# zsc/ARTalk

Measured on AMD Instinct MI355X. Metric: motion frames/sec (25 fps clips) at batch=32 per GPU, higher is better.
Workload: dtype f32 (operands split into 2 fp16, 3 fp16 MFMA products per fp32 product, fp32 accumulate)

## Files before the change

artalk_amd/capi.py:

```python
from __future__ import annotations

import ctypes as C
import os

from .config import ARTalkConfig

_HERE = os.path.dirname(os.path.abspath(__file__))
LIB_PATH = os.environ.get("ARTALK_LIB") or os.path.join(_HERE, "libartalk_hip.so")

OK, EINVAL, EKEY, EMISSING, EHIP, ESTATE, ECAPACITY, EBUSY = 0, -1, -2, -3, -4, -5, -6, -7
DTYPE_F32, DTYPE_I64 = 0, 1

SYMBOLS = [
    "artalk_create", "artalk_destroy", "artalk_last_error", "artalk_set_tensor", "artalk_finalize_weights",
    "artalk_reserve", "artalk_workspace_bytes", "artalk_weight_bytes", "artalk_infer", "artalk_get_status", "artalk_poll_status", "artalk_last_ticket", "artalk_get_status_of", "artalk_style_encode", "artalk_stream_begin", "artalk_stream_chunk", "artalk_stream_end", "artalk_savgol", "artalk_flame_create", "artalk_flame_verts", "artalk_flame_destroy", "artalk_flame_last_error",
    "artalk_set_profiling", "artalk_get_profile", "artalk_get_kernel_sums", "artalk_set_graphs", "artalk_graph_count", "artalk_set_cu_mask", "artalk_set_audit", "artalk_get_audit", "artalk_calibrate", "artalk_reset_scales", "artalk_get_scales", "artalk_scale_sites", "artalk_get_site_scales", "artalk_set_site_scales", "artalk_set_tap", "artalk_tap_layout", "artalk_set_precision",
    "artalk_op_gemm", "artalk_op_gemm_ex", "artalk_op_gemm_bf16", "artalk_op_gemm_f16s", "artalk_op_pack_split", "artalk_op_gemm_f16s_packed", "artalk_op_release_scratch", "artalk_op_gemm_p8_plan", "artalk_op_create_masked_stream", "artalk_op_destroy_stream", "artalk_op_mfma_f32_peak", "artalk_op_layernorm", "artalk_op_attention", "artalk_op_w2v_front", "artalk_op_resample_mean", "artalk_op_pool_silu",
    "artalk_op_bsq_history",
    "artalk_sessions_reserve", "artalk_session_open", "artalk_session_step", "artalk_session_close", "artalk_session_count",
    "artalk_op_pack_split_ex", "artalk_op_layernorm_ex", "artalk_op_gemm_f16s_packed_ex", "artalk_op_gemm_f16s_ex", "artalk_op_attention_ex", "artalk_op_w2v_front_ex", "artalk_op_pool_silu_ex", "artalk_op_posconv_p8_ex",
    "artalk_op_bsq_history_ex", "artalk_op_ar_bits_next", "artalk_op_vq_embed", "artalk_op_ar_begin", "artalk_op_dec_input", "artalk_op_dec_finish", "artalk_op_enc_input_zero", "artalk_op_style_input", "artalk_op_add_row", "artalk_op_style_finish", "artalk_op_broadcast16", "artalk_op_session_gather", "artalk_op_session_scatter", "artalk_op_absmax",
]


class ArtalkConfigStruct(C.Structure):
    _fields_ = [
        ("ar_depth", C.c_int32), ("ar_heads", C.c_int32),
        ("vae_depth", C.c_int32), ("vae_heads", C.c_int32), ("vae_hidden", C.c_int32),
        ("code_dim", C.c_int32), ("motion_dim", C.c_int32),
        ("n_levels", C.c_int32), ("patch_nums", C.c_int32 * 8),
        ("w2v_layers", C.c_int32), ("w2v_hidden", C.c_int32), ("w2v_heads", C.c_int32), ("w2v_ffn", C.c_int32),
        ("w2v_n_conv", C.c_int32), ("w2v_conv_kernel", C.c_int32 * 8), ("w2v_conv_stride", C.c_int32 * 8),
        ("w2v_conv_dim", C.c_int32),
        ("w2v_pos_kernel", C.c_int32), ("w2v_pos_groups", C.c_int32),
        ("w2v_ln_eps", C.c_float),
        ("style_dim", C.c_int32), ("style_heads", C.c_int32), ("style_layers", C.c_int32), ("style_ffn", C.c_int32),
        ("style_len", C.c_int32),
    ]


def config_struct(cfg: ARTalkConfig) -> ArtalkConfigStruct:
    w = cfg.w2v
    if w.get("feat_extract_norm", "layer") != "layer" or not w.get("do_stable_layer_norm", True) or not w.get("conv_bias", True):
        raise ValueError("only the XLS-R style wav2vec2 (layer-norm conv stack, stable layer norm, conv bias) is supported")
# ... 177 lines not shown
        L.artalk_op_w2v_front_ex.restype = i32
        L.artalk_op_pool_silu_ex.argtypes = [vp, i32, i32, i32, vp, i32, i32, vp, vp]
        L.artalk_op_pool_silu_ex.restype = i32
        L.artalk_op_posconv_p8_ex.argtypes = [vp, vp, vp, vp, vp, i32, i32, i32, i32, i32, vp, vp]
        L.artalk_op_posconv_p8_ex.restype = i32
    if hasattr(L, "artalk_op_ar_bits_next"):
        for name, args in (
                ("bsq_history_ex", [vp, vp, vp, vp, i32, vp, vp]),
                ("ar_bits_next", [vp, vp, vp, vp, i32, i32, vp, vp]),
                ("vq_embed", [vp, i32, vp, vp, vp, vp, i32, i32, vp, vp, i32, vp]),
                ("ar_begin", [vp, vp, vp, vp, i32, vp]),
                ("dec_input", [vp, vp, vp, vp, vp, i32, vp]),
                ("dec_finish", [vp, vp, vp, vp, vp, i64, i32, vp, i32, vp, vp]),
                ("enc_input_zero", [vp, vp, vp, vp, i32, vp]),
                ("style_input", [vp, vp, vp, vp, i32, vp]),
                ("add_row", [vp, vp, i32, i32, vp]),
                ("style_finish", [vp, vp, vp, vp, vp, vp, i32, vp, i64, vp]),
                ("broadcast16", [vp, vp, i64, i32, vp]),
                ("session_gather", [vp, vp, vp, vp, i32, i32, i32, i32, vp]),
                ("session_scatter", [vp, vp, vp, vp, i32, i32, i32, i32, i32, vp]),
                ("absmax", [vp, i32, i32, i64, i32, i32, i32, i32, vp, vp])):
            f = getattr(L, "artalk_op_" + name)
            f.argtypes, f.restype = args, i32
    _lib = L
    return L


def ptr(t):
    return None if t is None else C.c_void_p(t.data_ptr())


def current_stream_ptr():
    import torch
    return C.c_void_p(torch.cuda.current_stream().cuda_stream)
```

artalk_amd/csrc/ar_glue.hip:

```cpp
#include "common.h"
#include <cmath>
#include <mutex>
#include <set>

namespace artalk {

constexpr int T100 = 100;
constexpr int CD = 32;
constexpr int NLV = 5;
__constant__ int c_pn[NLV];
__constant__ int c_off[NLV + 1];
__constant__ int c_up_i0[4][T100];
__constant__ int c_up_i1[4][T100];
__constant__ float c_up_w1[4][T100];
__constant__ float c_hq;

static const int h_pn[NLV] = {1, 5, 25, 50, 100};

int init_ms_tables() {
    static std::mutex mu;
    static std::set<int> ready;
    int dev = -1;
    if (hipGetDevice(&dev) != hipSuccess) return -1;
    std::lock_guard<std::mutex> lock(mu);
// ... 95 lines not shown
        if (status && !(isfinite(l[0]) && isfinite(l[1]))) atomicOr(status, 1);
        bits[((long)b * 181 + off + i) * CD + c] = (uint8_t)bit;
        hs[idx] = bit ? c_hq : -c_hq;
    }
    if (p >= NLV - 1) return;
    __syncthreads();
    float* fg = fhat + (long)b * T100 * CD;
    for (int idx = tid; idx < T100 * CD; idx += BITS_NT) {
        const int t = idx / CD, c = idx % CD;
        const float v = fg[idx] + up_lin(hs, p, t, c);
        fg[idx] = v;
        fs[idx] = v;
    }
    __syncthreads();
    const int pn2 = c_pn[p + 1];
    for (int idx = tid; idx < pn2 * CD; idx += BITS_NT)
        nextfeat[(long)b * pn2 * CD + idx] = area_pool(fs, pn2, idx / CD, idx % CD);
}
void launch_ar_bits_next(const float* logits, uint8_t* bits, float* fhat, float* nextfeat, int B, int level, hipStream_t s, int* status) {
    ARTALK_LAUNCH(ar_bits_kernel, dim3(B), dim3(BITS_NT), 0, s, logits, bits, fhat, nextfeat, level, status);
}

constexpr int VQ_TOK = 16;
__global__ __launch_bounds__(256) void vq_embed_kernel(const float* __restrict__ feat, int n, const float* __restrict__ We,
                                                       const float* __restrict__ be, const float* __restrict__ pos,
                                                       float* __restrict__ X, int xrows, int xoff,
                                                       const float* __restrict__ style_cond, const float* __restrict__ pos0, int E) {
    __shared__ float f[VQ_TOK][CD];
    const int i0 = blockIdx.x * VQ_TOK, b = blockIdx.y, tid = threadIdx.x;
    if (blockIdx.x == 0 && style_cond) {
        for (int e = tid; e < E; e += 256) X[((long)b * xrows) * E + e] = style_cond[(long)b * E + e] + pos0[e];
    }
    const int nt = min(VQ_TOK, n - i0);
    for (int idx = tid; idx < VQ_TOK * CD; idx += 256) f[idx / CD][idx % CD] = idx < nt * CD ? feat[((long)b * n + i0) * CD + idx] : 0.f;
    constexpr int EPT = 3;
    float w[EPT][CD], bias[EPT], pv[EPT][VQ_TOK];
#pragma unroll
    for (int k = 0; k < EPT; ++k) {
        const int e = tid + k * 256;
        const bool ok = e < E;
#pragma unroll
        for (int c4 = 0; c4 < CD / 4; ++c4) {
            f32x4 t = {0.f, 0.f, 0.f, 0.f};
            if (ok) t = *reinterpret_cast<const f32x4*>(We + (long)e * CD + 4 * c4);
            w[k][4 * c4] = t[0]; w[k][4 * c4 + 1] = t[1]; w[k][4 * c4 + 2] = t[2]; w[k][4 * c4 + 3] = t[3];
        }
        bias[k] = ok ? be[e] : 0.f;
#pragma unroll
        for (int t = 0; t < VQ_TOK; ++t) pv[k][t] = (ok && t < nt) ? pos[(long)(i0 + t) * E + e] : 0.f;
    }
    __syncthreads();
#pragma unroll
    for (int k = 0; k < EPT; ++k) {
        const int e = tid + k * 256;
        if (e >= E) break;
#pragma unroll
        for (int t0 = 0; t0 < VQ_TOK; t0 += 4) {
            float acc[4] = {0.f, 0.f, 0.f, 0.f};
#pragma unroll
            for (int c = 0; c < CD; ++c)
#pragma unroll
                for (int u = 0; u < 4; ++u) acc[u] = fmaf(w[k][c], f[t0 + u][c], acc[u]);
#pragma unroll
            for (int u = 0; u < 4; ++u)
                if (t0 + u < nt) X[((long)b * xrows + xoff + i0 + t0 + u) * E + e] = (acc[u] + bias[k]) + pv[k][t0 + u];
        }
    }
}
void launch_vq_embed(const float* feat, int n, const float* We, const float* be, const float* pos, float* X, int xrows,
                     int xoff, const float* style_cond, const float* pos0, int B, hipStream_t s) {
    ARTALK_LAUNCH(vq_embed_kernel, dim3((n + VQ_TOK - 1) / VQ_TOK, B), dim3(256), 0, s, feat, n, We, be, pos, X, xrows, xoff,
                       style_cond, pos0, 768);
}

__global__ __launch_bounds__(256) void dec_input_kernel(const float* __restrict__ prev_fdec, const float* __restrict__ fhat,
                                                        const uint8_t* __restrict__ bits, const float* __restrict__ dpos,
                                                        float* __restrict__ X) {
    const int b = blockIdx.x;
    for (int idx = blockIdx.y * 256 + threadIdx.x; idx < 2 * T100 * CD; idx += gridDim.y * 256) {
        const int t = idx / CD, c = idx % CD;
        float v;
        if (t < T100) {
            v = prev_fdec[(long)b * T100 * CD + idx];
        } else {
            const int tt = t - T100;
            const float h = bits[((long)b * 181 + 81 + tt) * CD + c] ? c_hq : -c_hq;
            v = fhat[(long)b * T100 * CD + tt * CD + c] + h;
        }
        X[(long)b * 2 * T100 * CD + idx] = v + dpos[idx];
    }
}
void launch_dec_input(const float* prev_fdec, const float* fhat, const uint8_t* bits, const float* dpos, float* X, int B,
                      hipStream_t s) {
    ARTALK_LAUNCH(dec_input_kernel, dim3(B, 8), dim3(256), 0, s, prev_fdec, fhat, bits, dpos, X);
}
// ... 257 lines not shown
```

artalk_amd/csrc/engine.hip:

```cpp
#include "kernels.h"
#include "../../include/artalk_hip.h"

#include <hip/hip_ext.h>
#include <rocprofiler-sdk-roctx/roctx.h>

#include <algorithm>
#include <cmath>
#include <cstdio>
#include <cstdlib>
#include <cstring>
#include <map>
#include <set>
#include <string>
#include <vector>

using namespace artalk;

namespace artalk {
thread_local KernelTimer* g_ktimer = nullptr;
bool ktimer_events(hipEvent_t* e0, hipEvent_t* e1) {
    KernelTimer* t = g_ktimer;
    if (!t) return false;
    while (t->pool.size() < t->used + 2) {
        hipEvent_t e = nullptr;
// ... 88 lines not shown
    int64_t weight_bytes = 0;
    struct PackRange { const float* base; int64_t n; unsigned int* packed; uint16_t* bf16; };
    std::vector<PackRange> wranges;
    int precision = 0;
    bool have_bf16 = false;
    int splitk_tiles = 192, splitk_target = 384;
    bool audit = false;
    unsigned int* audit_vals = nullptr;
    std::vector<std::string> audit_names;
    std::map<std::string, int> audit_index;
    std::vector<int*> audit_exp;
    SiteExps ex;
    int scales_changed = 0;
    struct Site { std::string name; int* ex; };
    std::vector<Site> sites;
    std::map<const int*, int> site_of;
    bool stream_scales_ended = false;
    struct InitHistory { uint8_t* bits = nullptr; float *fdec = nullptr, *msfeat = nullptr; bool valid = false; } init_hist[3];
    void invalidate_init_hist() { for (auto& ih : init_hist) ih.valid = false; }
    float* tap = nullptr; int tap_B = 0, tap_maxch = 0, tap_chunk = 0;
    std::vector<uint32_t> cu_mask;
    int n_cus = 0;
    int stream_B = 0;
    static constexpr int kSessBlock = 32;
    struct Sessions {
        std::vector<float*> blocks;
        std::vector<int64_t> owner;
        std::map<int64_t, int> open;
        std::set<int64_t> ended_by_scales;
        int64_t next_id = 1;
    } sess;
    int64_t sess_slot_floats() const { return kE + (int64_t)kNTok * kE + 100LL * cfg.code_dim; }
    float* sess_slot(int i) const { return sess.blocks[i / kSessBlock] + (int64_t)(i % kSessBlock) * sess_slot_floats(); }
    Workspace* view = nullptr;
    bool sticky_error = false;
    int n_conv = 0; int conv_T[8]{}; int conv_S[8]{};
    int Tw = 0, Ts = 0;
    int ada_n = 0;
    int pn[kMaxLv]{}, off[kMaxLv + 1]{};
    float *conv0_w = nullptr, *conv_b[8]{}, *conv_lnw[8]{}, *conv_lnb[8]{}, *conv_w[8]{};
    float *fp_lnw = nullptr, *fp_lnb = nullptr, *fp_w = nullptr, *fp_b = nullptr;
    float *pos_w = nullptr, *pos_b = nullptr, *enc_lnw = nullptr, *enc_lnb = nullptr;
    std::vector<W2VLayer> w2v;
    float *ada_w = nullptr, *ada_b = nullptr;
    float *ar_qkv_w = nullptr, *ar_qkv_b = nullptr;
    std::vector<ARLayer> ar;
// ... 508 lines not shown
        SiteExps::VAE& E = m->ex.vae[sd][i];
        layernorm(w.vh, w.vln, L.lnw, L.lnb, M, H, 1e-5f, ACT_NONE, s, p8, w.status, 0, 0, E.ln);
        audit(m, w.vln, M, H, H, p8, s, &E.ln);
        linear(m, w.vln, H, L.qkv_w, nullptr, w.vqkv, 3 * H, M, 3 * H, H, ACT_NONE, nullptr, s, AP | (p8 ? LF_C_P8 : 0), nullptr, E.ln, E.qkv);
        AttnArgs a;
        a.qkv_p8 = p8; a.qkv_exp = E.qkv; a.o_exp = E.attn;
        a.Q = w.vqkv; a.K = w.vqkv + H; a.V = w.vqkv + 2 * H; a.ldq = a.ldk = a.ldv = 3 * H;
        a.q_bstride = a.k_bstride = a.v_bstride = (long)T * 3 * H;
        a.O = w.vatt; a.ldo = H; a.o_bstride = (long)T * H;
        a.B = B; a.H = c.vae_heads; a.HD = H / c.vae_heads; a.Lq = T; a.Lk = T;
        a.scale = 1.0f / std::sqrt((float)H);
        audit(m, w.vqkv, M, 3 * H, 3 * H, p8, s, &E.qkv);
        a.split_q = split; a.split_k = split; a.out_p8 = p8; a.split16 = p8; a.status = p8 ? w.status : nullptr; a.cus = m->n_cus;
        launch_attention(a, s);
        audit(m, w.vatt, M, H, H, p8, s, &E.attn);
        linear(m, w.vatt, H, L.out_w, L.out_b, w.vh, H, M, H, H, ACT_NONE, w.vh, s, AP, p8 ? w.vln : nullptr, E.attn, E.resid);
        audit(m, p8 ? w.vln : w.vh, M, H, H, p8, s, &E.resid);
        linear(m, p8 ? w.vln : w.vh, H, L.m1_w, L.m1_b, w.vmlp, F, M, F, H, ACT_GELU_TANH, nullptr, s, p8 ? (LF_A_P8 | LF_C_P8) : 0, nullptr, E.resid, E.mlp);
        audit(m, w.vmlp, M, F, F, p8, s, &E.mlp);
        linear(m, w.vmlp, F, L.m2_w, L.m2_b, w.vh, H, M, H, F, ACT_NONE, w.vh, s, AP, nullptr, E.mlp);
    }
}

void run_reencode(artalk_model* m, int B, hipStream_t s) {
    const artalk_config& c = m->cfg;
    Workspace& w = m->view ? *m->view : m->ws;
    const int H = c.vae_hidden, T = 100;
    Range r_re("artalk.vae.reencode_bsq");
    kbucket(m, KB_REENC);
    audit(m, w.enc_in, B * T, 128, 128, false, s, &m->ex.vae_enc_in);
    linear(m, w.enc_in, 128, m->enc.in_w, m->enc.in_b, w.vh, H, B * T, H, 128, ACT_LEAKY02, nullptr, s, 0, nullptr, m->ex.vae_enc_in);
    run_vae_stack(m, m->enc, B, T, 0, s);
    linear(m, w.vh, H, m->enc.out_w, m->enc.out_b, w.enc_out, c.code_dim, B * T, c.code_dim, H, ACT_NONE, nullptr, s, LF_EXACT);
    launch_bsq_history(w.enc_out, w.hist_bits, w.prev_fdec, w.msfeat, B, s, w.status);
    launch_vq_embed(w.msfeat, kNTok - 1, m->vq_w, m->vq_b, m->prev_lvl_pos + kE, w.prev_in, kNTok, 1, w.style_cond,
                    m->prev_lvl_pos, B, s);
}

int run_init_history(artalk_model* m, int B, hipStream_t s) {
    const artalk_config& c = m->cfg;
    struct Restore { artalk_model* m; ~Restore() { kbucket(m, KB_OTHER); } } restore{m};
    Workspace& w = m->ws;
    artalk_model::InitHistory& ih = m->init_hist[m->precision];
    const long nb = (long)kNTok * c.code_dim, nf = 100L * c.code_dim * 4, nm = 180L * c.code_dim * 4;
    if (!ih.valid) {
        if (!ih.bits) {
            ih.bits = dalloc<uint8_t>(m, nb); ih.fdec = dalloc<float>(m, nf / 4); ih.msfeat = dalloc<float>(m, nm / 4);
            if (!ih.bits || !ih.fdec || !ih.msfeat) return fail(m, ARTALK_EHIP, "hipMalloc failed for the initial-history cache");
            HIPCHK(m, hipDeviceSynchronize());
        }
        launch_enc_input_zero(m->vae_mean, m->vae_std, m->enc_pos, w.enc_in, 1, s);
        run_reencode(m, 1, s);
        HIPCHK(m, hipMemcpyAsync(ih.bits, w.hist_bits, nb, hipMemcpyDeviceToDevice, s));
        HIPCHK(m, hipMemcpyAsync(ih.fdec, w.prev_fdec, nf, hipMemcpyDeviceToDevice, s));
        HIPCHK(m, hipMemcpyAsync(ih.msfeat, w.msfeat, nm, hipMemcpyDeviceToDevice, s));
        int flags[4] = {0, 0, 0, 0};
        HIPCHK(m, hipMemcpyAsync(flags, w.status, sizeof(int), hipMemcpyDeviceToHost, s));
        HIPCHK(m, hipStreamSynchronize(s));
        ih.valid = flags[0] == 0;
    }
    launch_broadcast16(ih.bits, w.hist_bits, nb, B, s);
    launch_broadcast16(ih.fdec, w.prev_fdec, nf, B, s);
    launch_broadcast16(ih.msfeat, w.msfeat, nm, B, s);
    launch_vq_embed(w.msfeat, kNTok - 1, m->vq_w, m->vq_b, m->prev_lvl_pos + kE, w.prev_in, kNTok, 1, w.style_cond, m->prev_lvl_pos, B, s);
    return ARTALK_OK;
}

void run_chunk_body(artalk_model* m, int B, hipStream_t s, int n_reencode = -1) {
    struct BodyScope { artalk_model* m; BodyScope(artalk_model* x) : m(x) { m->in_body = true; } ~BodyScope() { m->in_body = false; } } scope(m);
    const artalk_config& c = m->cfg;
    Workspace& w = m->view ? *m->view : m->ws;
    const long ldada = m->ada_n;
    const long cache_l = (long)w.maxB * 2 * kNTok * 3 * kE;
    const int p8 = m->precision == 1 ? 1 : 0;
    kbucket(m, KB_AR_MISC);
    tap_copy(m, TAP_PREV_IN, 0, w.prev_in, kNTok, kE, B, s);
    roctxRangePushA("artalk.ar.history_kv");
    SiteExps& ex = m->ex;
    if (p8) launch_pack_split(w.prev_in, reinterpret_cast<unsigned int*>(w.prev_in_p8), (long)B * kNTok * kE, false, s, w.status, ex.hist_tok);
    audit(m, p8 ? w.prev_in_p8 : w.prev_in, B * kNTok, kE, kE, p8, s, &ex.hist_tok);
    {
        GemmArgs g;
        g.A = p8 ? w.prev_in_p8 : w.prev_in; g.a_packed = p8; g.a_exp = ex.hist_tok;
        g.lda = kE; g.W = m->ar_qkv_w + (long)kE * kE; g.ldw = kE; g.bias = m->ar_qkv_b + kE;
        g.C = w.cache + kE; g.ldc = 3 * kE; g.cmap = rowmap(kNTok, 2 * kNTok, 0);
        g.M = B * kNTok; g.N = c.ar_depth * 2 * kE; g.K = kE;
        g.ngrp = 2 * kE; g.grpW = (long)3 * kE * kE; g.grpB = 3 * kE; g.grpC = cache_l;
        g.Wp = packed_of(m, g.W);
        if (p8 && gemm_p8_eligible(g)) {
            gemm(m, g, s);
        } else {
            for (int l = 0; l < c.ar_depth; ++l) {
                const ARLayer& L = m->ar[l];
                GemmArgs q = g;
                q.Wp = nullptr; q.ngrp = 0; q.grpW = q.grpB = q.grpC = 0;
                q.W = L.qkv_w + (long)kE * kE; q.bias = L.qkv_b + kE; q.C = w.cache + l * cache_l + kE; q.N = 2 * kE;
                gemm(m, q, s);
            }
        }
    }
    roctxRangePop();
    launch_ar_begin(w.style_cond, m->lvl_pos, w.x, w.fhat, B, s);
// ... 38 lines not shown
            a.B = B; a.H = c.ar_heads; a.HD = kE / c.ar_heads; a.Lq = pn; a.Lk = kNTok + off + pn; a.scale = 1.0f;
            a.l2norm = 1; a.qscale = L.qscale; a.out_p8 = p8; a.split16 = p8; a.status = p8 ? w.status : nullptr; a.o_exp = E.attn;
            launch_attention(a, s);
            audit(m, w.attn_out, M, kE, kE, p8, s, &E.attn);
            GemmArgs pj;
            pj.A = w.attn_out; pj.lda = kE; pj.W = L.proj_w; pj.ldw = kE; pj.bias = L.proj_b; pj.C = w.x; pj.ldc = kE;
            pj.gate = ada; pj.ldg = ldada; pj.gmap = amap; pj.R = w.x; pj.ldr = kE; pj.M = M; pj.N = kE; pj.K = kE; pj.a_packed = p8; pj.a_exp = E.attn;
            const LnArgs n2 = ln_args(l, 1);
            if (!gemm(m, pj, s, &n2)) launch_layernorm(n2, s);
            audit(m, w.xmod, M, kE, kE, p8, s, &E.ln2);
            linear(m, w.xmod, kE, L.ffn1_w, L.ffn1_b, w.ffn_h, 4 * kE, M, 4 * kE, kE, ACT_GELU_TANH, nullptr, s, p8 ? (LF_A_P8 | LF_C_P8) : 0, nullptr, E.ln2, E.ffn);
            audit(m, w.ffn_h, M, 4 * kE, 4 * kE, p8, s, &E.ffn);
            GemmArgs f2;
            f2.A = w.ffn_h; f2.lda = 4 * kE; f2.W = L.ffn2_w; f2.ldw = 4 * kE; f2.bias = L.ffn2_b; f2.C = w.x; f2.ldc = kE;
            f2.gate = ada + kE; f2.ldg = ldada; f2.gmap = amap; f2.R = w.x; f2.ldr = kE; f2.M = M; f2.N = kE; f2.K = 4 * kE; f2.a_packed = p8; f2.a_exp = E.ffn;
            const LnArgs nn = ln_args(l + 1, 0);
            have_ln = gemm(m, f2, s, &nn);
            if (l == 0) tap_copy(m, TAP_BLK0_OUT, off, w.x, pn, kE, B, s);
            if (l == c.ar_depth - 1) tap_copy(m, TAP_BLKL_OUT, off, w.x, pn, kE, B, s);
        }
        if (!have_ln) launch_layernorm(ln_args(c.ar_depth, 0), s);
        linear(m, w.xmod, kE, m->logits_w, m->logits_b, w.logits, 2 * c.code_dim, M, 2 * c.code_dim, kE, ACT_NONE, nullptr, s, LF_EXACT);
        tap_copy(m, TAP_LOGITS, off, w.logits, pn, 2 * c.code_dim, B, s);
        launch_ar_bits_next(w.logits, w.bits, w.fhat, w.nextfeat, B, p, s, w.status);
        if (p + 1 < c.n_levels)
            launch_vq_embed(w.nextfeat, m->pn[p + 1], m->vq_w, m->vq_b, m->lvl_pos + (long)m->off[p + 1] * kE, w.x, m->pn[p + 1], 0,
                            nullptr, nullptr, B, s);
    }
    stage_mark(m, s, PB_AR);
    const int H = c.vae_hidden;
    roctxRangePushA("artalk.vae.decode");
    kbucket(m, KB_VAE_DEC);
    launch_dec_input(w.prev_fdec, w.fhat, w.bits, m->dec_pos, w.dec_x, B, s);
    audit(m, w.dec_x, B * 200, c.code_dim, c.code_dim, false, s, &ex.vae_dec_in);
    linear(m, w.dec_x, c.code_dim, m->dec.in_w, m->dec.in_b, w.vh, H, B * 200, H, c.code_dim, ACT_LEAKY02, nullptr, s, 0, nullptr, ex.vae_dec_in);
    run_vae_stack(m, m->dec, B, 200, 100, s);
    audit(m, w.vh, B * 200, H, H, false, s, &ex.vae_dec_head);
    linear(m, w.vh, H, m->dec.out_w, m->dec.out_b, w.dec_out, c.motion_dim, B * 200, c.motion_dim, H, ACT_NONE, nullptr, s, 0, nullptr, ex.vae_dec_head);
    tap_copy(m, TAP_DEC_OUT, 0, w.dec_out, 200, c.motion_dim, B, s);
    launch_dec_finish(w.dec_out, m->vae_mean, m->vae_std, m->enc_pos, w.motion_chunk, 100L * c.motion_dim, 0, w.enc_in, B, s, w.status);
    roctxRangePop();
    if (n_reencode < 0 || n_reencode > B) n_reencode = B;
    if (n_reencode > 0) run_reencode(m, n_reencode, s);
    stage_mark(m, s, PB_VAE);
}

Workspace clip_view(const artalk_model* m, int b0, int branch) {
    const artalk_config& c = m->cfg;
    Workspace v = m->ws;
    const long b = b0;
// ... 137 lines not shown
    return ARTALK_OK;
}
int publish_status(artalk_model* m, hipStream_t s) {
    const int slot = (int)(m->ticket % artalk_model::kStatusSlots);
    if (m->ticket >= artalk_model::kStatusSlots) HIPCHK(m, hipEventSynchronize(m->status_ev[slot]));
    HIPCHK(m, hipMemcpyAsync(m->h_status + slot, m->ws.status, sizeof(int), hipMemcpyDeviceToHost, s));
    HIPCHK(m, hipEventRecord(m->status_ev[slot], s));
    ++m->ticket;
    m->status_pending = true;
    HIPCHK(m, hipGetLastError());
    return ARTALK_OK;
}

int reserve(artalk_model* m, int maxB, int maxC) {
    const artalk_config& c = m->cfg;
    if (maxB <= m->ws.maxB && maxC <= m->ws.maxC) return ensure_stage(m, m->ws.maxB, m->ws.maxC);
    maxB = std::max(maxB, m->ws.maxB); maxC = std::max(maxC, m->ws.maxC);
    (void)hipDeviceSynchronize();
    drop_graphs(m);
    for (void* p : m->ws_allocs) if (p) (void)hipFree(p);
    m->ws_allocs.clear();
    m->ws = Workspace();
    m->stream_B = 0; m->stream_scales_ended = false;
    m->status_pending = false;
    Workspace& w = m->ws;
    const int CD = c.w2v_conv_dim, Hs = c.w2v_hidden;
    w.maxB = maxB; w.maxC = maxC; w.G = std::min(maxC, 96);
    auto F = [&](int64_t n) { w.bytes += n * 4; return dalloc_in<float>(m->ws_allocs, n); };
    const int G = w.G;
    w.src_off = dalloc_in<long>(m->ws_allocs, maxC);
    w.xnorm = F((int64_t)G * kSamplesPerChunk);
    w.convA = F(((int64_t)G * m->conv_S[0] + 16) * CD);
    w.convB = F(((int64_t)G * m->conv_S[1] + 16) * CD);
    const int64_t M = (int64_t)G * m->Ts;
    w.h0 = F(M * Hs); w.h1 = F(M * Hs); w.xln = F(M * Hs); w.qkv = F(M * 3 * Hs); w.att = F(M * Hs); w.ffn = F(M * c.w2v_ffn);
    w.silu_cond = F((int64_t)maxC * kNTok * kCond);
    w.ada = F((int64_t)maxB * kNTok * m->ada_n);
    w.style_cond = F((int64_t)maxB * kE);
    w.prev_in = F((int64_t)maxB * kNTok * kE); w.prev_in_p8 = F((int64_t)maxB * kNTok * kE);
    w.cache = F((int64_t)c.ar_depth * maxB * 2 * kNTok * 3 * kE);
    w.x = F((int64_t)maxB * 100 * kE); w.xmod = F((int64_t)maxB * 100 * kE); w.attn_out = F((int64_t)maxB * 100 * kE);
    w.ffn_h = F((int64_t)maxB * 100 * 4 * kE); w.logits = F((int64_t)maxB * 100 * 2 * c.code_dim);
    w.splitk_floats = (int64_t)8 << 20; w.splitk = F(w.splitk_floats); w.splitk_b[0] = w.splitk;
    for (int i = 1; i < 4; ++i) w.splitk_b[i] = F(w.splitk_floats);
    w.fhat = F((int64_t)maxB * 100 * c.code_dim); w.nextfeat = F((int64_t)maxB * 100 * c.code_dim);
    w.bits = dalloc_in<uint8_t>(m->ws_allocs, (int64_t)maxB * kNTok * c.code_dim);
// ... 96 lines not shown
    Workspace& w = m->ws;
    if (!has_style) style_motion_dev = nullptr;
    if (style_motion_dev) {
        std::memcpy(stg->has, has_style, (size_t)B);
        HIPCHK(m, hipMemcpyAsync(w.has_style, stg->has, B, hipMemcpyHostToDevice, s));
    }
    HIPCHK(m, hipEventRecord(stg->done, s));
    stg->used = true;
    HIPCHK(m, hipMemsetAsync(w.status, 0, 4 * sizeof(int), s));
    stage_mark(m, s, PB_OTHER);
    run_style(m, style_motion_dev, B, s, encode_style);
    stage_mark(m, s, PB_STYLE);
    return ARTALK_OK;
}
int chunk_step(artalk_model* m, hipStream_t s, int cond_row0, int Bn, int n_next, int tap_chunk, float* out_motion_dev, int64_t out_stride) {
    Workspace& w = m->ws;
    m->tap_chunk = tap_chunk;
    roctxRangePushA("artalk.ar.adaln_table");
    kbucket(m, KB_ADA);
    linear(m, w.silu_cond + (long)cond_row0 * kNTok * kCond, kCond, m->ada_w, m->ada_b, w.ada, m->ada_n, Bn * kNTok, m->ada_n, kCond,
           ACT_NONE, nullptr, s, m->precision == 1 ? LF_A_P8 : 0, nullptr, m->ex.silu_cond);
    roctxRangePop();
    stage_mark(m, s, PB_ADA);
    if (body_uses_graphs(m)) {
        Range r_body("artalk.body.graph");
        if (int rc = run_body(m, Bn, s, n_next)) return rc;
        stage_mark(m, s, PB_AR);
    } else {
        if (int rc = run_body(m, Bn, s, n_next)) return rc;
    }
    const size_t mrow = (size_t)100 * m->cfg.motion_dim * 4;
    HIPCHK(m, hipMemcpy2DAsync(out_motion_dev, (size_t)out_stride * 4, w.motion_chunk, mrow, mrow, Bn, hipMemcpyDeviceToDevice, s));
    return ARTALK_OK;
}

SessionRows session_rows(const artalk_model* m) {
    const Workspace& w = m->ws;
    SessionRows r;
    r.style = reinterpret_cast<uint4*>(w.style_cond); r.prev_in = reinterpret_cast<uint4*>(w.prev_in); r.prev_fdec = reinterpret_cast<uint4*>(w.prev_fdec);
    r.s16 = kE / 4; r.p16 = kNTok * kE / 4; r.f16 = 100 * m->cfg.code_dim / 4;
    return r;
}
int grow_sessions(artalk_model* m, int64_t n_slots) {
    artalk_model::Sessions& ss = m->sess;
    if (m->cfg.code_dim % 4) return fail(m, ARTALK_EINVAL, "sessions need a code_dim that is a multiple of 4 (16-byte rows)");
    while ((int64_t)ss.owner.size() < n_slots) {
        void* p = nullptr;
        HIPCHK(m, hipMalloc(&p, (size_t)artalk_model::kSessBlock * m->sess_slot_floats() * sizeof(float)));
        ss.blocks.push_back(static_cast<float*>(p));
        ss.owner.resize(ss.owner.size() + artalk_model::kSessBlock, 0);
    }
    return ARTALK_OK;
}
// ... 546 lines not shown
            if (ss.ended_by_scales.count(ids[i]))
                return fail(m, ARTALK_ESTATE, "session " + std::to_string(ids[i]) + ": the site scales changed since artalk_session_open; open the session again");
            return fail(m, ARTALK_EINVAL, "artalk_session_step: " + std::to_string(ids[i]) + " is not an open session");
        }
        if (!seen.insert(ids[i]).second) return fail(m, ARTALK_EINVAL, "artalk_session_step: session " + std::to_string(ids[i]) + " is listed twice");
        slot[i] = it->second;
    }
    hipStream_t s;
    if (int rc = call_stream(m, stream, &s)) return rc;
    if (n > m->ws.maxB || n > m->ws.maxC) { if (int rc = reserve(m, n, n)) return rc; }
    Workspace& w = m->ws;
    artalk_model::Stage* stg = nullptr;
    if (int rc = next_stage(m, &stg)) return rc;
    for (int b = 0; b < n; ++b) stg->src[b] = (long)b * chunk_stride;
    HIPCHK(m, hipMemcpyAsync(w.src_off, stg->src, n * sizeof(long), hipMemcpyHostToDevice, s));
    if (int rc = stage_session_slots(m, s, stg, slot.data(), n)) return rc;
    HIPCHK(m, hipEventRecord(stg->done, s));
    stg->used = true;
    m->stream_B = 0; m->stream_scales_ended = false;
    HIPCHK(m, hipMemsetAsync(w.status, 0, 4 * sizeof(int), s));
    const SessionRows rows = session_rows(m);
    ProfilingOff quiet(m);
    launch_session_gather(w.sess_slots, rows, n, s);
    for (int c0 = 0; c0 < n; c0 += w.G) run_wav2vec(m, audio_dev, c0, std::min(w.G, n - c0), nullptr, s);
    if (int rc = chunk_step(m, s, 0, n, n, m->tap_maxch, out_motion_dev, out_stride)) return rc;
    launch_session_scatter(w.sess_slots, rows, n, false, s);
    const size_t bits_n = (size_t)n * kNTok * m->cfg.code_dim;
    if (out_bits_dev) HIPCHK(m, hipMemcpyAsync(out_bits_dev, w.bits, bits_n, hipMemcpyDeviceToDevice, s));
    if (out_hist_bits_dev) HIPCHK(m, hipMemcpyAsync(out_hist_bits_dev, w.hist_bits, bits_n, hipMemcpyDeviceToDevice, s));
    if (int rc = publish_status(m, s)) return rc;
    return ARTALK_OK;
}

int artalk_session_close(artalk_model* m, const int64_t* ids, int n) {
    if (!m || !ids || n <= 0) return ARTALK_EINVAL;
    artalk_model::Sessions& ss = m->sess;
    std::set<int64_t> seen;
    for (int i = 0; i < n; ++i)
        if ((!ss.open.count(ids[i]) && !ss.ended_by_scales.count(ids[i])) || !seen.insert(ids[i]).second)
            return fail(m, ARTALK_EINVAL, "artalk_session_close: " + std::to_string(ids[i]) + " is not an open session (or is listed twice)");
    for (int i = 0; i < n; ++i) {
        const auto it = ss.open.find(ids[i]);
        if (it != ss.open.end()) { ss.owner[it->second] = 0; ss.open.erase(it); }
        ss.ended_by_scales.erase(ids[i]);
    }
    return ARTALK_OK;
// ... 341 lines not shown
    return artalk_op_bsq_history_ex(enc_out, hist_bits, prev_fdec, msfeat, B, nullptr, stream);
}
int artalk_op_bsq_history_ex(const float* enc_out, uint8_t* hist_bits, float* prev_fdec, float* msfeat, int B, int* status_dev, void* stream) {
    if (!enc_out || !hist_bits || !prev_fdec || !msfeat || B <= 0) return ARTALK_EINVAL;
    if (init_ms_tables() != 0) return ARTALK_EHIP;
    launch_bsq_history(enc_out, hist_bits, prev_fdec, msfeat, B, (hipStream_t)stream, status_dev);
    return hipGetLastError() == hipSuccess ? ARTALK_OK : ARTALK_EHIP;
}

int artalk_op_ar_bits_next(const float* logits, uint8_t* bits, float* fhat, float* nextfeat, int B, int level, int* status_dev, void* stream) {
    if (!logits || !bits || B <= 0 || level < 0 || level > 4 || (level < 4 && (!fhat || !nextfeat))) return ARTALK_EINVAL;
    if (init_ms_tables() != 0) return ARTALK_EHIP;
    launch_ar_bits_next(logits, bits, fhat, nextfeat, B, level, (hipStream_t)stream, status_dev);
    return hipGetLastError() == hipSuccess ? ARTALK_OK : ARTALK_EHIP;
}
int artalk_op_vq_embed(const float* feat, int n, const float* We, const float* be, const float* pos, float* X, int xrows, int xoff,
                       const float* style_cond, const float* pos0, int B, void* stream) {
    if (!feat || !We || !be || !pos || !X || n <= 0 || B <= 0 || xoff < 0 || xrows < xoff + n) return ARTALK_EINVAL;
    if (style_cond && (!pos0 || xoff < 1)) return ARTALK_EINVAL;
    if (((uintptr_t)We) & 15) return ARTALK_EINVAL;
    launch_vq_embed(feat, n, We, be, pos, X, xrows, xoff, style_cond, pos0, B, (hipStream_t)stream);
    return hipGetLastError() == hipSuccess ? ARTALK_OK : ARTALK_EHIP;
}
int artalk_op_ar_begin(const float* style_cond, const float* lvlpos, float* x0, float* fhat, int B, void* stream) {
    if (!style_cond || !lvlpos || !x0 || !fhat || B <= 0) return ARTALK_EINVAL;
    launch_ar_begin(style_cond, lvlpos, x0, fhat, B, (hipStream_t)stream);
    return hipGetLastError() == hipSuccess ? ARTALK_OK : ARTALK_EHIP;
}
int artalk_op_dec_input(const float* prev_fdec, const float* fhat, const uint8_t* bits, const float* dpos, float* X, int B, void* stream) {
    if (!prev_fdec || !fhat || !bits || !dpos || !X || B <= 0) return ARTALK_EINVAL;
    if (init_ms_tables() != 0) return ARTALK_EHIP;
    launch_dec_input(prev_fdec, fhat, bits, dpos, X, B, (hipStream_t)stream);
    return hipGetLastError() == hipSuccess ? ARTALK_OK : ARTALK_EHIP;
}
int artalk_op_dec_finish(const float* dec, const float* mean, const float* std_, const float* epos, float* out, int64_t out_bstride,
                         int chunk, float* E, int B, int* status_dev, void* stream) {
    if (!dec || !mean || !std_ || !epos || !out || !E || B <= 0 || chunk < 0) return ARTALK_EINVAL;
    if (out_bstride < ((int64_t)chunk + 1) * 100 * 106) return ARTALK_EINVAL;
    launch_dec_finish(dec, mean, std_, epos, out, (long)out_bstride, chunk, E, B, (hipStream_t)stream, status_dev);
    return hipGetLastError() == hipSuccess ? ARTALK_OK : ARTALK_EHIP;
}
int artalk_op_enc_input_zero(const float* mean, const float* std_, const float* epos, float* E, int B, void* stream) {
    if (!mean || !std_ || !epos || !E || B <= 0) return ARTALK_EINVAL;
    launch_enc_input_zero(mean, std_, epos, E, B, (hipStream_t)stream);
    return hipGetLastError() == hipSuccess ? ARTALK_OK : ARTALK_EHIP;
}
// ... 149 lines not shown
```

artalk_amd/csrc/kernels.h:

```cpp
#pragma once
#include <hip/hip_runtime.h>
#include <climits>
#include <cstdint>

#include <hip/hip_ext.h>
#include <utility>
#include <vector>

namespace artalk {

struct KernelTimer {
    int bucket = 0;
    std::vector<hipEvent_t> pool; size_t used = 0;
    std::vector<std::pair<int, size_t>> recs;
};
extern thread_local KernelTimer* g_ktimer;
bool ktimer_events(hipEvent_t* e0, hipEvent_t* e1);
#define ARTALK_LAUNCH(kernel, grid, block, lds, stream, ...)                                                          \
    do {                                                                                                              \
        hipEvent_t kt_e0_ = nullptr, kt_e1_ = nullptr;                                                                \
        if (artalk::g_ktimer && artalk::ktimer_events(&kt_e0_, &kt_e1_))                                              \
            hipExtLaunchKernelGGL(kernel, grid, block, lds, stream, kt_e0_, kt_e1_, 0, __VA_ARGS__);                  \
        else                                                                                                          \
            hipLaunchKernelGGL(kernel, grid, block, lds, stream, __VA_ARGS__);                                        \
// ... 87 lines not shown
    int B = 0, H = 0, HD = 64, Lq = 0, Lk = 0;
    float scale = 1.f;
    int l2norm = 0; const float* qscale = nullptr;
    int split_q = 0, split_k = 0;
    int out_p8 = 0;
    int split16 = 0;
    int qkv_p8 = 0;
    int qkv_exp = 4, o_exp = 4;
    int* status = nullptr;
    int cus = 0;
};
void launch_attention(const AttnArgs& a, hipStream_t s);
void attention_prepare();

void launch_audio_normalize(const float* audio, const long* src_off, float* xnorm, int n_chunks, int n, hipStream_t s);
void launch_conv0(const float* xnorm, int n, const float* w , const float* bias, const float* lnw,
                  const float* lnb, float* Y, int n_chunks, int T, int row_stride, hipStream_t s, int out_p8 = 0, int* status = nullptr, int p8_exp = kActExp);
void launch_pool_silu(const float* X, int x_tstride, int T, float* Y, int n_chunks, const int* patch_nums, int n_lvls,
                      int D, hipStream_t s, int out_p8 = 0, int* status = nullptr, int p8_exp = kActExp);

void launch_ar_bits_next(const float* logits, uint8_t* bits, float* fhat, float* nextfeat, int B, int level, hipStream_t s,
                         int* status = nullptr);
void launch_vq_embed(const float* feat, int n, const float* We, const float* be, const float* pos, float* X, int xrows,
                     int xoff, const float* style_cond, const float* pos0, int B, hipStream_t s);
void launch_ar_begin(const float* style_cond, const float* lvlpos, float* x0, float* fhat, int B, hipStream_t s);
void launch_dec_input(const float* prev_fdec, const float* fhat, const uint8_t* bits, const float* dpos, float* X,
                      int B, hipStream_t s);
void launch_dec_finish(const float* dec , const float* mean, const float* stdv, const float* epos,
                       float* out, long out_bstride, int chunk, float* E, int B, hipStream_t s, int* status = nullptr);
void launch_enc_input_zero(const float* mean, const float* stdv, const float* epos, float* E, int B, hipStream_t s);
void launch_broadcast16(const void* src, void* dst, long bytes, int B, hipStream_t s);
struct SessionRows {
    uint4* style; uint4* prev_in; uint4* prev_fdec;
    int s16, p16, f16;
};
void launch_session_gather(const float* const* slots, const SessionRows& w, int n, hipStream_t s);
void launch_session_scatter(float* const* slots, const SessionRows& w, int n, bool with_style, hipStream_t s);
void launch_bsq_history(const float* enc_out, uint8_t* hist_bits, float* prev_fdec, float* msfeat, int B, hipStream_t s,
                        int* status = nullptr);
void launch_style_input(const float* motion, const float* mean, const float* stdv, float* X, int B, hipStream_t s);
void launch_style_finish(const float* feat , const float* Ws, const float* bs, const float* null_cond,
                         const uint8_t* has_style, float* style_cond, int B, hipStream_t s, const float* cached = nullptr,
                         long cached_stride = 0);
void launch_add_row(float* X, const float* v, int M, int D, hipStream_t s);
void launch_savgol(const float* in, float* out, int T, int D, hipStream_t s);

double launch_mfma_f32_peak(float* out, int blocks, int iters, int nacc, hipStream_t s);
// ... 12 lines not shown
```

include/artalk_hip.h:

```cpp
#ifndef ARTALK_HIP_H
#define ARTALK_HIP_H

#include <stdint.h>

#ifdef __cplusplus
extern "C" {
#endif

#define ARTALK_OK 0
#define ARTALK_EINVAL (-1)
#define ARTALK_EKEY (-2)
#define ARTALK_EMISSING (-3)
#define ARTALK_EHIP (-4)
#define ARTALK_ESTATE (-5)
#define ARTALK_ECAPACITY (-6)
#define ARTALK_EBUSY (-7)

#define ARTALK_DTYPE_F32 0
#define ARTALK_DTYPE_I64 1

typedef struct artalk_model artalk_model;

typedef struct artalk_config {
    int32_t ar_depth, ar_heads;
// ... 95 lines not shown
int artalk_op_pool_silu(const float* X, int C, int T, int D, float* Y, void* stream);
int artalk_op_pack_split_ex(const float* in, void* out_u32, int64_t n, int is_weight, int p8_exp, int* status_dev, void* stream);
int artalk_op_layernorm_ex(const float* X, float* Y, const float* w, const float* b, const float* scale, const float* shift,
                           int M, int D, float eps, int act, int p8_exp, int junk_period, int junk_from, int* status_dev, void* stream);
int artalk_op_gemm_f16s_packed_ex(const void* A, int a_packed, int64_t lda, const void* Wp, const float* bias, float* C, int M, int N,
                                  int K, int act, int force_cfg, int a_exp, int c_exp, void* c2_u32, int* status_dev, void* stream);
int artalk_op_gemm_f16s_ex(const float* A, int64_t lda, const float* W, const float* bias, float* C, int M, int N, int K, int act,
                           int force_cfg, int a_exp, int* status_dev, void* stream);
int artalk_op_attention_ex(const float* Q, const float* K, const float* V, float* O, int B, int H, int HD, int Lq, int Lk,
                           float scale, int l2norm, const float* qscale, int split, int qkv_exp, int o_exp, int out_p8,
                           int* status_dev, void* stream);
int artalk_op_w2v_front_ex(const float* audio, int C, int n, const float* w, const float* bias, const float* lnw,
                           const float* lnb, float* xnorm_out, float* Y, int out_p8, int p8_exp, int* status_dev, void* stream);
int artalk_op_pool_silu_ex(const float* X, int C, int T, int D, float* Y, int out_p8, int p8_exp, int* status_dev, void* stream);
int artalk_op_posconv_p8_ex(const float* X, const void* Wp, const float* bias, const float* R, float* C, int n_chunks, int T, int Ts,
                            int act, int a_exp, int* status_dev, void* stream);
int artalk_op_bsq_history(const float* enc_out, uint8_t* hist_bits, float* prev_fdec, float* msfeat, int B, void* stream);
int artalk_op_bsq_history_ex(const float* enc_out, uint8_t* hist_bits, float* prev_fdec, float* msfeat, int B, int* status_dev,
                             void* stream);
int artalk_op_ar_bits_next(const float* logits, uint8_t* bits, float* fhat, float* nextfeat, int B, int level, int* status_dev,
                           void* stream);
int artalk_op_vq_embed(const float* feat, int n, const float* We, const float* be, const float* pos, float* X, int xrows, int xoff,
                       const float* style_cond, const float* pos0, int B, void* stream);
int artalk_op_ar_begin(const float* style_cond, const float* lvlpos, float* x0, float* fhat, int B, void* stream);
int artalk_op_dec_input(const float* prev_fdec, const float* fhat, const uint8_t* bits, const float* dpos, float* X, int B, void* stream);
int artalk_op_dec_finish(const float* dec, const float* mean, const float* std_, const float* epos, float* out, int64_t out_bstride,
                         int chunk, float* E, int B, int* status_dev, void* stream);
int artalk_op_enc_input_zero(const float* mean, const float* std_, const float* epos, float* E, int B, void* stream);
int artalk_op_style_input(const float* motion, const float* mean, const float* std_, float* X, int B, void* stream);
int artalk_op_add_row(float* X, const float* v, int M, int D, void* stream);
int artalk_op_style_finish(const float* feat, const float* Ws, const float* bs, const float* null_cond, const uint8_t* has_style,
                           float* style_cond, int B, const float* cached, int64_t cached_stride, void* stream);
int artalk_op_broadcast16(const void* src, void* dst, int64_t bytes, int B, void* stream);
int artalk_op_session_gather(const float* const* slots_dev, float* style, float* prev_in, float* prev_fdec, int s16, int p16, int f16, int n,
                             void* stream);
int artalk_op_session_scatter(float* const* slots_dev, const float* style, const float* prev_in, const float* prev_fdec, int s16, int p16,
                              int f16, int n, int with_style, void* stream);
int artalk_op_absmax(const float* buf, int rows, int cols, int64_t ld, int is_p8, int p8_exp, int junk_period, int junk_from,
                     unsigned int* slot_dev, void* stream);

#ifdef __cplusplus
}
#endif
#endif
```

Measured before the change: 101,100.

## Fuse AR bit decode with next-level VQ embed and emit packed history in embed

Replaces the per-level ar_bits_next plus vq_embed pair with one ar_tail kernel. Each block decodes bits, updates its slice of fhat, pools the next-level features and embeds them without a round trip through global memory. The history embedding kernel now also writes the split-fp16 packed copy directly, and a cached exponent tracker skips the separate pack_split pass when the packed history is already current. The fused kernel makes each block redo the logit decode for its level, and the cache-validity tracking adds state that could go stale if invalidation is missed.

```diff
diff --git a/artalk_amd/capi.py b/artalk_amd/capi.py
--- a/artalk_amd/capi.py
+++ b/artalk_amd/capi.py
@@ -20,6 +20,7 @@
     "artalk_sessions_reserve", "artalk_session_open", "artalk_session_step", "artalk_session_close", "artalk_session_count",
     "artalk_op_pack_split_ex", "artalk_op_layernorm_ex", "artalk_op_gemm_f16s_packed_ex", "artalk_op_gemm_f16s_ex", "artalk_op_attention_ex", "artalk_op_w2v_front_ex", "artalk_op_pool_silu_ex", "artalk_op_posconv_p8_ex",
     "artalk_op_bsq_history_ex", "artalk_op_ar_bits_next", "artalk_op_vq_embed", "artalk_op_ar_begin", "artalk_op_dec_input", "artalk_op_dec_finish", "artalk_op_enc_input_zero", "artalk_op_style_input", "artalk_op_add_row", "artalk_op_style_finish", "artalk_op_broadcast16", "artalk_op_session_gather", "artalk_op_session_scatter", "artalk_op_absmax",
+    "artalk_op_vq_embed_p8", "artalk_op_ar_tail",
 ]
 
 
@@ -243,6 +244,11 @@
                 ("absmax", [vp, i32, i32, i64, i32, i32, i32, i32, vp, vp])):
             f = getattr(L, "artalk_op_" + name)
             f.argtypes, f.restype = args, i32
+    if hasattr(L, "artalk_op_ar_tail"):
+        L.artalk_op_vq_embed_p8.argtypes = [vp, i32, vp, vp, vp, vp, vp, i32, i32, vp, vp, i32, i32, vp, vp]
+        L.artalk_op_vq_embed_p8.restype = i32
+        L.artalk_op_ar_tail.argtypes = [vp, vp, vp, vp, i32, i32, vp, vp, vp, vp, vp, vp]
+        L.artalk_op_ar_tail.restype = i32
     _lib = L
     return L
 
diff --git a/artalk_amd/csrc/ar_glue.hip b/artalk_amd/csrc/ar_glue.hip
--- a/artalk_amd/csrc/ar_glue.hip
+++ b/artalk_amd/csrc/ar_glue.hip
@@ -141,14 +141,27 @@
 }
 
 constexpr int VQ_TOK = 16;
+__device__ __forceinline__ void store_p8x1(float* row, int e, float v, int* status, int p8_exp) {
+    p8_guard(status, v, 0.f, 0.f, 0.f, p8_maxbits_of(p8_exp));
+    _Float16 hh, ll;
+    split_f16(v * p8_scale_of(p8_exp), hh, ll);
+    _Float16* g = reinterpret_cast<_Float16*>(row) + (e >> 3) * 16 + (e & 7);
+    g[0] = hh;
+    g[8] = ll;
+}
 __global__ __launch_bounds__(256) void vq_embed_kernel(const float* __restrict__ feat, int n, const float* __restrict__ We,
                                                        const float* __restrict__ be, const float* __restrict__ pos,
                                                        float* __restrict__ X, int xrows, int xoff,
-                                                       const float* __restrict__ style_cond, const float* __restrict__ pos0, int E) {
+                                                       const float* __restrict__ style_cond, const float* __restrict__ pos0, int E,
+                                                       float* __restrict__ Xp8, int p8_exp, int* __restrict__ status) {
     __shared__ float f[VQ_TOK][CD];
     const int i0 = blockIdx.x * VQ_TOK, b = blockIdx.y, tid = threadIdx.x;
     if (blockIdx.x == 0 && style_cond) {
-        for (int e = tid; e < E; e += 256) X[((long)b * xrows) * E + e] = style_cond[(long)b * E + e] + pos0[e];
+        for (int e = tid; e < E; e += 256) {
+            const float v = style_cond[(long)b * E + e] + pos0[e];
+            X[((long)b * xrows) * E + e] = v;
+            if (Xp8) store_p8x1(Xp8 + ((long)b * xrows) * E, e, v, status, p8_exp);
+        }
     }
     const int nt = min(VQ_TOK, n - i0);
     for (int idx = tid; idx < VQ_TOK * CD; idx += 256) f[idx / CD][idx % CD] = idx < nt * CD ? feat[((long)b * n + i0) * CD + idx] : 0.f;
@@ -182,14 +195,92 @@
                 for (int u = 0; u < 4; ++u) acc[u] = fmaf(w[k][c], f[t0 + u][c], acc[u]);
 #pragma unroll
             for (int u = 0; u < 4; ++u)
-                if (t0 + u < nt) X[((long)b * xrows + xoff + i0 + t0 + u) * E + e] = (acc[u] + bias[k]) + pv[k][t0 + u];
+                if (t0 + u < nt) {
+                    const long row = ((long)b * xrows + xoff + i0 + t0 + u) * E;
+                    const float v = (acc[u] + bias[k]) + pv[k][t0 + u];
+                    X[row + e] = v;
+                    if (Xp8) store_p8x1(Xp8 + row, e, v, status, p8_exp);
+                }
         }
     }
 }
 void launch_vq_embed(const float* feat, int n, const float* We, const float* be, const float* pos, float* X, int xrows,
-                     int xoff, const float* style_cond, const float* pos0, int B, hipStream_t s) {
+                     int xoff, const float* style_cond, const float* pos0, int B, hipStream_t s, float* Xp8, int p8_exp, int* status) {
     ARTALK_LAUNCH(vq_embed_kernel, dim3((n + VQ_TOK - 1) / VQ_TOK, B), dim3(256), 0, s, feat, n, We, be, pos, X, xrows, xoff,
-                       style_cond, pos0, 768);
+                       style_cond, pos0, 768, Xp8, p8_exp, status);
+}
+
+constexpr int TAIL_NT = 768;
+__global__ __launch_bounds__(TAIL_NT) void ar_tail_kernel(const float* __restrict__ logits, uint8_t* __restrict__ bits,
+                                                          float* __restrict__ fhat, float* __restrict__ nextfeat, int p,
+                                                          int* __restrict__ status, const float* __restrict__ We,
+                                                          const float* __restrict__ be, const float* __restrict__ pos,
+                                                          float* __restrict__ X, int E) {
+    __shared__ float hs[50 * CD];
+    __shared__ float fs[T100 * CD];
+    __shared__ float f[VQ_TOK][CD];
+    const int b = blockIdx.y, tid = threadIdx.x;
+    const int pn = c_pn[p], off = c_off[p], pn2 = c_pn[p + 1];
+    const int i0 = blockIdx.x * VQ_TOK, nt = min(VQ_TOK, pn2 - i0);
+    const int fw = T100 / pn2, t0 = i0 * fw, nfr = nt * fw;
+    const int e = tid;
+    const bool eok = e < E;
+    float w[CD], bias, pv[VQ_TOK];
+#pragma unroll
+    for (int c4 = 0; c4 < CD / 4; ++c4) {
+        f32x4 t = {0.f, 0.f, 0.f, 0.f};
+        if (eok) t = *reinterpret_cast<const f32x4*>(We + (long)e * CD + 4 * c4);
+        w[4 * c4] = t[0]; w[4 * c4 + 1] = t[1]; w[4 * c4 + 2] = t[2]; w[4 * c4 + 3] = t[3];
+    }
+    bias = eok ? be[e] : 0.f;
+#pragma unroll
+    for (int t = 0; t < VQ_TOK; ++t) pv[t] = (eok && t < nt) ? pos[(long)(i0 + t) * E + e] : 0.f;
+
+    for (int idx = tid; idx < pn * CD; idx += TAIL_NT) {
+        const int i = idx / CD, c = idx % CD;
+        const float* l = logits + ((long)b * pn + i) * (2 * CD) + 2 * c;
+        const int bit = l[1] > l[0];
+        if (blockIdx.x == 0) {
+            if (status && !(isfinite(l[0]) && isfinite(l[1]))) atomicOr(status, 1);
+            bits[((long)b * 181 + off + i) * CD + c] = (uint8_t)bit;
+        }
+        hs[idx] = bit ? c_hq : -c_hq;
+    }
+    __syncthreads();
+    float* fg = fhat + (long)b * T100 * CD + (long)t0 * CD;
+    for (int idx = tid; idx < nfr * CD; idx += TAIL_NT) {
+        const int t = t0 + idx / CD, c = idx % CD;
+        const float v = fg[idx] + up_lin(hs, p, t, c);
+        fg[idx] = v;
+        fs[idx] = v;
+    }
+    __syncthreads();
+    for (int idx = tid; idx < VQ_TOK * CD; idx += TAIL_NT) {
+        float v = 0.f;
+        if (idx < nt * CD) {
+            v = area_pool(fs, pn2, idx / CD, idx % CD);
+            nextfeat[((long)b * pn2 + i0) * CD + idx] = v;
+        }
+        f[idx / CD][idx % CD] = v;
+    }
+    __syncthreads();
+    if (!eok) return;
+#pragma unroll
+    for (int tk = 0; tk < VQ_TOK; tk += 2) {
+        float acc[2] = {0.f, 0.f};
+#pragma unroll
+        for (int c = 0; c < CD; ++c)
+#pragma unroll
+            for (int u = 0; u < 2; ++u) acc[u] = fmaf(w[c], f[tk + u][c], acc[u]);
+#pragma unroll
+        for (int u = 0; u < 2; ++u)
+            if (tk + u < nt) X[((long)b * pn2 + i0 + tk + u) * E + e] = (acc[u] + bias) + pv[tk + u];
+    }
+}
+void launch_ar_tail(const float* logits, uint8_t* bits, float* fhat, float* nextfeat, int B, int level, const float* We, const float* be,
+                    const float* pos, float* X, hipStream_t s, int* status) {
+    ARTALK_LAUNCH(ar_tail_kernel, dim3((h_pn[level + 1] + VQ_TOK - 1) / VQ_TOK, B), dim3(TAIL_NT), 0, s, logits, bits, fhat, nextfeat, level,
+                  status, We, be, pos, X, 768);
 }
 
 __global__ __launch_bounds__(256) void dec_input_kernel(const float* __restrict__ prev_fdec, const float* __restrict__ fhat,
diff --git a/artalk_amd/csrc/engine.hip b/artalk_amd/csrc/engine.hip
--- a/artalk_amd/csrc/engine.hip
+++ b/artalk_amd/csrc/engine.hip
@@ -134,6 +134,7 @@
     std::vector<uint32_t> cu_mask;
     int n_cus = 0;
     int stream_B = 0;
+    int hist_p8_exp = INT_MIN;
     static constexpr int kSessBlock = 32;
     struct Sessions {
         std::vector<float*> blocks;
@@ -688,6 +689,9 @@
     }
 }
 
+static float* hist_p8(const artalk_model* m, const Workspace& w) { return m->precision == 1 ? w.prev_in_p8 : nullptr; }
+static void hist_p8_written(artalk_model* m) { m->hist_p8_exp = m->precision == 1 ? m->ex.hist_tok : INT_MIN; }
+
 void run_reencode(artalk_model* m, int B, hipStream_t s) {
     const artalk_config& c = m->cfg;
     Workspace& w = m->view ? *m->view : m->ws;
@@ -700,7 +704,7 @@
     linear(m, w.vh, H, m->enc.out_w, m->enc.out_b, w.enc_out, c.code_dim, B * T, c.code_dim, H, ACT_NONE, nullptr, s, LF_EXACT);
     launch_bsq_history(w.enc_out, w.hist_bits, w.prev_fdec, w.msfeat, B, s, w.status);
     launch_vq_embed(w.msfeat, kNTok - 1, m->vq_w, m->vq_b, m->prev_lvl_pos + kE, w.prev_in, kNTok, 1, w.style_cond,
-                    m->prev_lvl_pos, B, s);
+                    m->prev_lvl_pos, B, s, hist_p8(m, w), m->ex.hist_tok, w.status);
 }
 
 int run_init_history(artalk_model* m, int B, hipStream_t s) {
@@ -728,7 +732,9 @@
     launch_broadcast16(ih.bits, w.hist_bits, nb, B, s);
     launch_broadcast16(ih.fdec, w.prev_fdec, nf, B, s);
     launch_broadcast16(ih.msfeat, w.msfeat, nm, B, s);
-    launch_vq_embed(w.msfeat, kNTok - 1, m->vq_w, m->vq_b, m->prev_lvl_pos + kE, w.prev_in, kNTok, 1, w.style_cond, m->prev_lvl_pos, B, s);
+    launch_vq_embed(w.msfeat, kNTok - 1, m->vq_w, m->vq_b, m->prev_lvl_pos + kE, w.prev_in, kNTok, 1, w.style_cond, m->prev_lvl_pos, B, s,
+                    hist_p8(m, w), m->ex.hist_tok, w.status);
+    hist_p8_written(m);
     return ARTALK_OK;
 }
 
@@ -743,7 +749,6 @@
     tap_copy(m, TAP_PREV_IN, 0, w.prev_in, kNTok, kE, B, s);
     roctxRangePushA("artalk.ar.history_kv");
     SiteExps& ex = m->ex;
-    if (p8) launch_pack_split(w.prev_in, reinterpret_cast<unsigned int*>(w.prev_in_p8), (long)B * kNTok * kE, false, s, w.status, ex.hist_tok);
     audit(m, p8 ? w.prev_in_p8 : w.prev_in, B * kNTok, kE, kE, p8, s, &ex.hist_tok);
     {
         GemmArgs g;
@@ -828,10 +833,10 @@
         if (!have_ln) launch_layernorm(ln_args(c.ar_depth, 0), s);
         linear(m, w.xmod, kE, m->logits_w, m->logits_b, w.logits, 2 * c.code_dim, M, 2 * c.code_dim, kE, ACT_NONE, nullptr, s, LF_EXACT);
         tap_copy(m, TAP_LOGITS, off, w.logits, pn, 2 * c.code_dim, B, s);
-        launch_ar_bits_next(w.logits, w.bits, w.fhat, w.nextfeat, B, p, s, w.status);
         if (p + 1 < c.n_levels)
-            launch_vq_embed(w.nextfeat, m->pn[p + 1], m->vq_w, m->vq_b, m->lvl_pos + (long)m->off[p + 1] * kE, w.x, m->pn[p + 1], 0,
-                            nullptr, nullptr, B, s);
+            launch_ar_tail(w.logits, w.bits, w.fhat, w.nextfeat, B, p, m->vq_w, m->vq_b, m->lvl_pos + (long)m->off[p + 1] * kE, w.x, s, w.status);
+        else
+            launch_ar_bits_next(w.logits, w.bits, w.fhat, w.nextfeat, B, p, s, w.status);
     }
     stage_mark(m, s, PB_AR);
     const int H = c.vae_hidden;
@@ -1015,6 +1020,7 @@
     m->ws_allocs.clear();
     m->ws = Workspace();
     m->stream_B = 0; m->stream_scales_ended = false;
+    m->hist_p8_exp = INT_MIN;
     m->status_pending = false;
     Workspace& w = m->ws;
     const int CD = c.w2v_conv_dim, Hs = c.w2v_hidden;
@@ -1157,6 +1163,8 @@
            ACT_NONE, nullptr, s, m->precision == 1 ? LF_A_P8 : 0, nullptr, m->ex.silu_cond);
     roctxRangePop();
     stage_mark(m, s, PB_ADA);
+    if (m->precision == 1 && m->hist_p8_exp != m->ex.hist_tok)
+        launch_pack_split(w.prev_in, reinterpret_cast<unsigned int*>(w.prev_in_p8), (long)Bn * kNTok * kE, false, s, w.status, m->ex.hist_tok);
     if (body_uses_graphs(m)) {
         Range r_body("artalk.body.graph");
         if (int rc = run_body(m, Bn, s, n_next)) return rc;
@@ -1164,6 +1172,7 @@
     } else {
         if (int rc = run_body(m, Bn, s, n_next)) return rc;
     }
+    hist_p8_written(m);
     const size_t mrow = (size_t)100 * m->cfg.motion_dim * 4;
     HIPCHK(m, hipMemcpy2DAsync(out_motion_dev, (size_t)out_stride * 4, w.motion_chunk, mrow, mrow, Bn, hipMemcpyDeviceToDevice, s));
     return ARTALK_OK;
@@ -1756,6 +1765,7 @@
     const SessionRows rows = session_rows(m);
     ProfilingOff quiet(m);
     launch_session_gather(w.sess_slots, rows, n, s);
+    m->hist_p8_exp = INT_MIN;
     for (int c0 = 0; c0 < n; c0 += w.G) run_wav2vec(m, audio_dev, c0, std::min(w.G, n - c0), nullptr, s);
     if (int rc = chunk_step(m, s, 0, n, n, m->tap_maxch, out_motion_dev, out_stride)) return rc;
     launch_session_scatter(w.sess_slots, rows, n, false, s);
@@ -2143,6 +2153,22 @@
     launch_vq_embed(feat, n, We, be, pos, X, xrows, xoff, style_cond, pos0, B, (hipStream_t)stream);
     return hipGetLastError() == hipSuccess ? ARTALK_OK : ARTALK_EHIP;
 }
+int artalk_op_vq_embed_p8(const float* feat, int n, const float* We, const float* be, const float* pos, float* X, float* X_p8, int xrows,
+                          int xoff, const float* style_cond, const float* pos0, int B, int p8_exp, int* status_dev, void* stream) {
+    if (!feat || !We || !be || !pos || !X || !X_p8 || n <= 0 || B <= 0 || xoff < 0 || xrows < xoff + n) return ARTALK_EINVAL;
+    if (style_cond && (!pos0 || xoff < 1)) return ARTALK_EINVAL;
+    if ((((uintptr_t)We) & 15) || (((uintptr_t)X_p8) & 31) || !op_exp_ok(p8_exp)) return ARTALK_EINVAL;
+    launch_vq_embed(feat, n, We, be, pos, X, xrows, xoff, style_cond, pos0, B, (hipStream_t)stream, X_p8, p8_exp, status_dev);
+    return hipGetLastError() == hipSuccess ? ARTALK_OK : ARTALK_EHIP;
+}
+int artalk_op_ar_tail(const float* logits, uint8_t* bits, float* fhat, float* nextfeat, int B, int level, const float* We, const float* be,
+                      const float* pos, float* X, int* status_dev, void* stream) {
+    if (!logits || !bits || !fhat || !nextfeat || !We || !be || !pos || !X || B <= 0 || level < 0 || level > 3) return ARTALK_EINVAL;
+    if (((uintptr_t)We) & 15) return ARTALK_EINVAL;
+    if (init_ms_tables() != 0) return ARTALK_EHIP;
+    launch_ar_tail(logits, bits, fhat, nextfeat, B, level, We, be, pos, X, (hipStream_t)stream, status_dev);
+    return hipGetLastError() == hipSuccess ? ARTALK_OK : ARTALK_EHIP;
+}
 int artalk_op_ar_begin(const float* style_cond, const float* lvlpos, float* x0, float* fhat, int B, void* stream) {
     if (!style_cond || !lvlpos || !x0 || !fhat || B <= 0) return ARTALK_EINVAL;
     launch_ar_begin(style_cond, lvlpos, x0, fhat, B, (hipStream_t)stream);
diff --git a/artalk_amd/csrc/kernels.h b/artalk_amd/csrc/kernels.h
--- a/artalk_amd/csrc/kernels.h
+++ b/artalk_amd/csrc/kernels.h
@@ -133,7 +133,10 @@
 void launch_ar_bits_next(const float* logits, uint8_t* bits, float* fhat, float* nextfeat, int B, int level, hipStream_t s,
                          int* status = nullptr);
 void launch_vq_embed(const float* feat, int n, const float* We, const float* be, const float* pos, float* X, int xrows,
-                     int xoff, const float* style_cond, const float* pos0, int B, hipStream_t s);
+                     int xoff, const float* style_cond, const float* pos0, int B, hipStream_t s, float* Xp8 = nullptr,
+                     int p8_exp = kActExp, int* status = nullptr);
+void launch_ar_tail(const float* logits, uint8_t* bits, float* fhat, float* nextfeat, int B, int level, const float* We, const float* be,
+                    const float* pos, float* X, hipStream_t s, int* status = nullptr);
 void launch_ar_begin(const float* style_cond, const float* lvlpos, float* x0, float* fhat, int B, hipStream_t s);
 void launch_dec_input(const float* prev_fdec, const float* fhat, const uint8_t* bits, const float* dpos, float* X,
                       int B, hipStream_t s);
diff --git a/include/artalk_hip.h b/include/artalk_hip.h
--- a/include/artalk_hip.h
+++ b/include/artalk_hip.h
@@ -141,6 +141,10 @@
                            void* stream);
 int artalk_op_vq_embed(const float* feat, int n, const float* We, const float* be, const float* pos, float* X, int xrows, int xoff,
                        const float* style_cond, const float* pos0, int B, void* stream);
+int artalk_op_vq_embed_p8(const float* feat, int n, const float* We, const float* be, const float* pos, float* X, float* X_p8, int xrows,
+                          int xoff, const float* style_cond, const float* pos0, int B, int p8_exp, int* status_dev, void* stream);
+int artalk_op_ar_tail(const float* logits, uint8_t* bits, float* fhat, float* nextfeat, int B, int level, const float* We, const float* be,
+                      const float* pos, float* X, int* status_dev, void* stream);
 int artalk_op_ar_begin(const float* style_cond, const float* lvlpos, float* x0, float* fhat, int B, void* stream);
 int artalk_op_dec_input(const float* prev_fdec, const float* fhat, const uint8_t* bits, const float* dpos, float* X, int B, void* stream);
 int artalk_op_dec_finish(const float* dec, const float* mean, const float* std_, const float* epos, float* out, int64_t out_bstride,
```

New measurement: 101,200, median of 6. No clear change (+0.1%).
